# pyannote/pyannote-video

Hardware: AMD Instinct MI355X
Metric: frames/sec end-to-end detect->embed->cluster, 1080p@25fps (higher is better)
Workload: dtype f32 (detector scores, embedder) / f64 (tracker, clustering) / u8 frames; an f16 screening pass with a proven error bound decides which windows the detector's exact f32 chain is evaluated for -- results identical to dense f32 scoring (`dense_scoring`)

## Files before the change

pyannote-video_amd/csrc/api.hip:

```cpp
#include "pvf_internal.h"
#include <algorithm>
#include <cmath>
#include <cstdlib>
#include <string>
#include <thread>

#define API_BEGIN try {
#define API_END                                                        \
    return 0;                                                          \
    }                                                                  \
    catch (const std::exception& e) { pvf_set_error(e.what()); return -1; } \
    catch (...) { pvf_set_error("unknown error"); return -2; }

#define ENTER(c, h)                                                \
    Ctx* c = pvf_ctx(h);                                           \
    std::lock_guard<std::recursive_mutex> _api_lock(c->api_mu);    \
    HIP_CHECK(hipSetDevice(c->device))
#define ENTER_DET(c, h)                                            \
    Ctx* c = pvf_ctx(h);                                           \
    std::lock_guard<std::recursive_mutex> _det_lock(c->det_mu);    \
    HIP_CHECK(hipSetDevice(c->device))
#define ENTER_BOTH(c, h)                                           \
    Ctx* c = pvf_ctx(h);                                           \
    std::lock_guard<std::recursive_mutex> _det_lock(c->det_mu);    \
// ... 37 lines not shown
    API_BEGIN
    ENTER_DET(c, h);
    if (batches) *batches = c->screen_batches;
    if (listed) *listed = c->screen_listed;
    if (retries) *retries = c->screen_retries;
    if (bounds) for (int f = 0; f < c->det.n_filters; ++f) bounds[f] = c->det.screen_bound[f];
    if (pipe_err) *pipe_err = c->screen_pipe_err;
    API_END
}

extern "C" int32_t pvf_embedder_split(pvf_handle h, int32_t on)
{
    API_BEGIN
    ENTER(c, h);
    c->emb_split = on != 0;
    API_END
}

extern "C" int32_t pvf_embedder_split_stats(pvf_handle h, int64_t* faces, int64_t* reruns, double* pipe_err)
{
    API_BEGIN
    ENTER(c, h);
    if (faces) *faces = c->emb_split_faces;
    if (reruns) *reruns = c->emb_reruns;
    if (pipe_err) *pipe_err = c->emb_pipe_err;
    API_END
}

extern "C" int32_t pvf_detect_batch(pvf_handle h, const pvf_handle* frames, int32_t n_frames, int32_t upsample, double adjust,
                                    pvf_rect_i32* out, float* scores, int32_t* counts, int32_t cap)
// ... 762 lines not shown
        const size_t bytes = (size_t)n * 150 * 150 * 3;
        c->s_trk0.ensure(bytes);
        HIP_CHECK(hipMemcpyAsync(c->s_trk0.p, chips, bytes, hipMemcpyHostToDevice, c->stream));
    }
    resnet_debug_stage(c, c->s_trk0.as<uint8_t>(), n, split != 0, &tap, flags);
    for (int i = 0; i < 3; ++i) dims[i] = tap.dims[i];
    API_END
}

extern "C" int32_t pvf_debug_conv(pvf_handle h, const int32_t geom[18], const float* in, const float* w, const float* bias, const float* gamma,
                                  const float* beta, const float* skip, int32_t split, int32_t force_generic, float* out, int32_t* flags)
{
    API_BEGIN
    ENTER(c, h);
    PVF_REQUIRE(geom, "pvf_debug_conv: bad arguments");
    resnet_debug_conv(c, geom, in, w, bias, gamma, beta, skip, split != 0, force_generic != 0, out, flags);
    API_END
}

extern "C" int32_t pvf_debug_embed_head(pvf_handle h, const float* x, int32_t n, int32_t hw, float* out)
{
    API_BEGIN
    ENTER(c, h);
    resnet_debug_head(c, x, n, hw, out);
    API_END
}

static PairInput table_f64(const double* X) { PairInput in; in.X = X; return in; }
static PairOutput host_full(double* D) { PairOutput o; o.out = D; return o; }

extern "C" int32_t pvf_pair_mean_dist(pvf_handle h, const double* X, int32_t N, int32_t dim, const int32_t* row_start, int32_t T, double* D)
// ... 375 lines not shown
```

pyannote-video_amd/csrc/ctx.hip:

```cpp
#include "pvf_internal.h"
#include "detect_ml.h"
#include <cmath>
#include <fstream>
#include <mutex>
#include <dlfcn.h>

static thread_local std::string g_err;
void pvf_set_error(const char* msg) { g_err = msg ? msg : ""; }
extern "C" const char* pvf_last_error(void) { return g_err.c_str(); }

static std::mutex g_ctx_mu;
static std::unordered_map<uint64_t, std::unique_ptr<Ctx>> g_ctxs;
static uint64_t g_next_ctx = 0x1000;

Ctx* pvf_ctx(pvf_handle h)
{
    std::lock_guard<std::mutex> lk(g_ctx_mu);
    auto it = g_ctxs.find(h);
    if (it == g_ctxs.end()) throw PvfError("unknown context handle");
    return it->second.get();
}

std::map<std::string, Tensor> pvf_read_container(const char* path)
{
// ... 272 lines not shown
    if (strncmp(prop.gcnArchName, "gfx950", 6) != 0)
        throw PvfError(std::string("libpvface is built for gfx950 (MI355X) only; device is ") + prop.gcnArchName);
    std::unique_ptr<Ctx> c(new Ctx());
    c->device = device;
    c->n_cu = prop.multiProcessorCount;
    {
        int lo = 0, hi = 0;
        HIP_CHECK(hipDeviceGetStreamPriorityRange(&lo, &hi));
        int prio = priority_class < 0 ? lo : hi;
        if (const char* e = getenv("PVF_MAIN_STREAM_PRIO")) prio = (strcmp(e, "low") == 0) ? lo : hi;
        HIP_CHECK(hipStreamCreateWithPriority(&c->stream, hipStreamNonBlocking, priority_class == 2 ? lo : prio));
        HIP_CHECK(hipStreamCreateWithPriority(&c->det_stream, hipStreamNonBlocking, priority_class == 2 ? hi : lo));
    }
    if (const char* e = getenv("PVF_DETECTOR_SCREENING")) c->det_screen = atoi(e) != 0;
    if (const char* e = getenv("PVF_EMBEDDER_SPLIT")) c->emb_split = atoi(e) != 0;
    std::lock_guard<std::mutex> lk(g_ctx_mu);
    uint64_t id = g_next_ctx++;
    g_ctxs[id] = std::move(c);
    *out = id;
    API_END
}

extern "C" int32_t pvf_ctx_create(int32_t device, pvf_handle* out) { return pvf_ctx_create_prio(device, 0, out); }

extern "C" int32_t pvf_ctx_destroy(pvf_handle h)
{
    API_BEGIN
    Ctx* c = pvf_ctx(h);
    HIP_CHECK(hipSetDevice(c->device));
    (void)hipStreamSynchronize(c->stream);
// ... 259 lines not shown
```

pyannote-video_amd/csrc/pvf_internal.h:

```cpp
#pragma once
#include <hip/hip_runtime.h>
#include <cstdint>
#include <cstdio>
#include <cstring>
#include <deque>
#include <map>
#include <atomic>
#include <memory>
#include <mutex>
#include <stdexcept>
#include <string>
#include <unordered_map>
#include <vector>
#include "../../include/pvface.h"
#include "scratch_layout.h"
#include "chip_plan.h"
#include "group_blocks.h"

#define PVF_FHOG_STRIDE 32

struct CandOverflow : PvfError { int needed; explicit CandOverflow(int n) : PvfError("detector: candidate buffer overflow"), needed(n) {} };
struct ScreenRetry : PvfError { ScreenRetry() : PvfError("detector: screening pass gave up") {} };

#define HIP_CHECK(expr)                                                                              \
// ... 194 lines not shown
    HostBuf h_cand, h_misc;
    StageRing stage;
    DevBuf s_cand2[2], s_fptr[2];
    HostBuf h_cand2[2], h_fptr[2];
    hipEvent_t det_ev[2] = {nullptr, nullptr};
    int det_slot = 0;
    int det_cand_cap = 8192;
    bool det_screen = true, det_screen_suspended = false, screen_attr_set = false;
    int screen_list_cap = 1 << 20;
    DevBuf s_screen;
    int64_t screen_batches = 0, screen_listed = 0, screen_retries = 0;
    double screen_pipe_err = -1;
    bool screen_pipe_flushes_subnormals = false;
    bool emb_split = true, emb_probe_done = false;
    DevBuf s_emb_flags, s_emb_redo;
    DevBuf s_jit;
    bool jit_attr_set = false;
    int64_t emb_split_faces = 0, emb_reruns = 0;
    double emb_pipe_err = -1;
    int n_cu = 256;
    struct PoolBuf { uint8_t* p; hipEvent_t free_after; hipEvent_t free_after_det; };
    std::map<size_t, std::deque<PoolBuf>> frame_pool;
    size_t frame_pool_bytes = 0;
    void* ingest_rings = nullptr;
    void* render_state = nullptr;
    void* tube_state = nullptr;
    void* board_state = nullptr;
    struct MlPlanCache* ml_plans = nullptr;
    std::map<std::vector<int>, std::unique_ptr<DevBuf>> resize_tabs;
    const void* feat_ring_owner = nullptr;
// ... 110 lines not shown
void dlib_mean_face_shape(float* out );
void resnet_forward(Ctx* c, const uint8_t* d_chips, int n, float* h_out);
struct ChipSource { const uint8_t* host; const pvf_handle* frames; const int32_t* pts; };
const EmbedModel& faces_geometry();
void faces_make_chips(Ctx* c, const pvf_handle* frames, const int32_t* pts, int m, uint8_t* d_chips);
void faces_source_round(Ctx* c, const ChipSource& src, int i0, int m, uint8_t* d_chips);
void sheet_check(const std::string& w, int W, int H, uint32_t background, const pvf_prim* prims, int n_prims, const uint8_t* text,
                 int64_t text_bytes, const uint8_t* rgb);
void sheet_prims_launch(Ctx* c, const pvf_prim* d_prims, int n_prims, const uint8_t* d_text, int W, int H, uint8_t* d_rgb);
void conv_layer_upload(ConvLayer& L, const float* w, const float* bias, const float* gamma, const float* beta);
void conv_layer_free(ConvLayer& L);
#define EMB_STAGES 30
struct EmbedTap { int stage; float* h_out; int dims[3]; };
void resnet_debug_stage(Ctx* c, const uint8_t* d_chips, int n, bool split, EmbedTap* tap, int* h_flags);
void resnet_debug_conv(Ctx* c, const int32_t* geom, const float* in, const float* w, const float* bias, const float* gamma, const float* beta,
                       const float* skip, bool split, bool force_generic, float* out, int32_t* flags);
void resnet_debug_head(Ctx* c, const float* x, int n, int hw, float* out);
void dsst_start_many(Ctx* c, const std::vector<Tracker*>& t, const std::vector<Frame>& f, const double* boxes);
void dsst_clone_many(Ctx* c, const std::vector<Tracker*>& src, const std::vector<Tracker*>& dst);
double* tracker_state_alloc(Ctx* c);
void shot_dfd(Ctx* c, const std::vector<Frame>& frames, int ow, int oh, const float* tables22, double* dfd, uint8_t* gray_out, float* flow_out);
void shot_run(Ctx* c, const std::vector<Frame>& frames, int ow, int oh, const float* tables22, double* dfd, uint8_t* gray_out, float* flow_out,
              int64_t* motion_rows);
void motion_fit_device(Ctx* c, const float* d_flow, int n_pairs, int h, int w, const double* d_dfd, int64_t* d_rows);
std::vector<int> orb_level_quota();
void orb_extract(Ctx* c, const std::vector<Frame>& frames, int ow, int oh, int cap, int32_t* counts, float* kp_out, uint8_t* desc_out);
void orb_match_counts(Ctx* c, const uint8_t* desc, const int32_t* nrows, int n_sets, int cap, const int32_t* pairs, int64_t n_pairs, int32_t* out);
void dsst_update_many(Ctx* c, const std::vector<Tracker*>& t, const std::vector<Frame>& f, double* psr, double* boxes_out, int mode = 0);
void overlap_matrix_host(const double* a, int na, const double* b, int nb, double ratio, double* out);
void munkres_host(const double* cost, int n, int32_t* row_to_col);
struct PairInput {
// ... 32 lines not shown
```

pyannote-video_amd/csrc/resnet.hip:

```cpp
#include "pvf_internal.h"
#include <cmath>
#include <cstdlib>
#include <cstring>
#include <vector>

typedef float f32x4 __attribute__((ext_vector_type(4)));
typedef uint32_t u32x4 __attribute__((ext_vector_type(4)));
typedef float f32x16 __attribute__((ext_vector_type(16)));
typedef _Float16 f16x8 __attribute__((ext_vector_type(8)));
typedef _Float16 f16x4 __attribute__((ext_vector_type(4)));
typedef uint32_t u32x2 __attribute__((ext_vector_type(2)));

void face_chip_details(const EmbedModel& m, const int32_t* pts, ChipDetails* out)
{
    const double size = m.chip_size, padding = m.chip_padding;
    double fx[51], fy[51], tx[51], ty[51];
    int n = 0;
    for (int i = 17; i < 68; ++i) {
        if ((55 <= i && i <= 59) || (65 <= i && i <= 67)) continue;
        if (17 <= i && i <= 26) continue;
        fx[n] = ((padding + (double)m.mean_shape[2 * (i - 17)]) / (2 * padding + 1)) * size;
        fy[n] = ((padding + (double)m.mean_shape[2 * (i - 17) + 1]) / (2 * padding + 1)) * size;
        tx[n] = pts[2 * i]; ty[n] = pts[2 * i + 1];
        ++n;
// ... 18 lines not shown
    out->cs = ca / scale; out->sn = cb / scale;
    out->rows = m.chip_size; out->cols = m.chip_size;
}

struct ConvArgs {
    const float* in; int B, H, W, Cin;
    const float* w; int K;
    const float* frag;
    const float* bias; const float* gamma; const float* beta;
    float* out; int OH, OW, Cout;
    int AH, AW;
    int ksz, stride, pad;
    int skip_mode;
    const float* skip; int XH, XW, XC, SH, SW;
    const uint32_t* wsplit; float out_scale; int* flags;
};


__device__ __forceinline__ int small_div(int x, int d, float rd)
{
    int q = (int)((float)x * rd);
    const int r = x - q * d;
    q += (r >= d) ? 1 : 0;
    q -= (r < 0) ? 1 : 0;
    return q;
}

template <int WM, int WN>
__device__ __forceinline__ void conv_epilogue(const ConvArgs& a, float* smem, const f32x16& acc0, const f32x16& acc1, long M, long m0, int n0,
                                              int rel0, int b_first, int hw, float r_hw, float r_ow, int wave, int lane)
{
    constexpr int PITCH = 36;
// ... 13 lines not shown
        const float4 bias4 = *reinterpret_cast<const float4*>(a.bias + cb), g4 = *reinterpret_cast<const float4*>(a.gamma + cb),
                     bt4 = *reinterpret_cast<const float4*>(a.beta + cb);
#pragma unroll
        for (int it = 0; it < 8; ++it) {
            const int row = it * 8 + (lane >> 3);
            const long m = m0 + wm * 64 + row;
            if (m >= M) continue;
            const float4 x = *reinterpret_cast<const float4*>(&T[row * PITCH + 4 * c4]);
            float4 v = make_float4((x.x + bias4.x) * g4.x + bt4.x, (x.y + bias4.y) * g4.y + bt4.y, (x.z + bias4.z) * g4.z + bt4.z,
                                   (x.w + bias4.w) * g4.w + bt4.w);
            if (a.skip_mode == 1) {
                const float4 sk = *reinterpret_cast<const float4*>(a.skip + (size_t)m * a.Cout + cb);
                v.x += sk.x; v.y += sk.y; v.z += sk.z; v.w += sk.w;
            }
            { v.x = v.x < 0.0f ? 0.0f : v.x; v.y = v.y < 0.0f ? 0.0f : v.y; v.z = v.z < 0.0f ? 0.0f : v.z; v.w = v.w < 0.0f ? 0.0f : v.w; }
            *reinterpret_cast<float4*>(a.out + (size_t)m * a.Cout + cb) = v;
        }
        return;
    }
#pragma unroll
    for (int t = 0; t < 2; ++t)
#pragma unroll
        for (int reg = 0; reg < 16; ++reg) {
            const int row = (reg & 3) + 8 * (reg >> 2) + 4 * kh;
            const long m = m0 + wm * 64 + t * 32 + row;
            if (m >= M) continue;
            const int rel = rel0 + wm * 64 + t * 32 + row;
            const int bb = small_div(rel, hw, r_hw);
            const int rem = rel - bb * hw;
            const int oy = small_div(rem, a.OW, r_ow);
            const int ox = rem - oy * a.OW;
// ... 29 lines not shown
#pragma unroll
        for (int q = 0; q < 4; ++q) {
            fa0[q] = *reinterpret_cast<const f32x4*>(pa0 + 4 * q);
            fa1[q] = *reinterpret_cast<const f32x4*>(pa1 + 4 * q);
            fb[q] = *reinterpret_cast<const f32x4*>(pb + 4 * q);
        }
#pragma unroll
        for (int s = 0; s < 16; ++s) {
            acc0 = __builtin_amdgcn_mfma_f32_32x32x2f32(fa0[s >> 2][s & 3], fb[s >> 2][s & 3], acc0, 0, 0, 0);
            acc1 = __builtin_amdgcn_mfma_f32_32x32x2f32(fa1[s >> 2][s & 3], fb[s >> 2][s & 3], acc1, 0, 0, 0);
        }
    }
    static __device__ __forceinline__ void scale(const ConvArgs&, f32x16&, f32x16&) {}
};

#define EMB_A_SCALE_EXP 8
#define EMB_F16_LIMIT 65504.0f
struct ConvSplit {
    static constexpr bool FLAGS = true;
    static constexpr int LANE_K = 4;
    static __device__ __forceinline__ const u32x4* weights(const ConvArgs& a) { return reinterpret_cast<const u32x4*>(a.wsplit); }
    static __device__ __forceinline__ bool park_a(uint32_t* row, int j4, const u32x4& v)
    {
        const f32x4 xv = __builtin_bit_cast(f32x4, v) * (float)(1 << EMB_A_SCALE_EXP);
        const bool ok = __builtin_reduce_and(__builtin_elementwise_abs(xv) < EMB_F16_LIMIT);
        const f16x4 hi = __builtin_convertvector(xv, f16x4), lo = __builtin_convertvector(xv - __builtin_convertvector(hi, f32x4), f16x4);
        *reinterpret_cast<u32x2*>(row + 2 * j4) = __builtin_bit_cast(u32x2, hi);
        *reinterpret_cast<u32x2*>(row + 2 * j4 + 16) = __builtin_bit_cast(u32x2, lo);
        return ok;
    }
    static __device__ __forceinline__ void park_b(uint32_t* row, int j4, const u32x4& v) { *reinterpret_cast<u32x4*>(row + 4 * j4) = v; }
    static __device__ __forceinline__ void chunk(const uint32_t* pa0, const uint32_t* pa1, const uint32_t* pb, f32x16& acc0, f32x16& acc1)
    {
#pragma unroll
        for (int s = 0; s < 2; ++s) {
            const f16x8 ah0 = *reinterpret_cast<const f16x8*>(pa0 + 8 * s), al0 = *reinterpret_cast<const f16x8*>(pa0 + 16 + 8 * s);
            const f16x8 ah1 = *reinterpret_cast<const f16x8*>(pa1 + 8 * s), al1 = *reinterpret_cast<const f16x8*>(pa1 + 16 + 8 * s);
            const f16x8 bh = *reinterpret_cast<const f16x8*>(pb + 8 * s), bl = *reinterpret_cast<const f16x8*>(pb + 16 + 8 * s);
            acc0 = __builtin_amdgcn_mfma_f32_32x32x16_f16(ah0, bh, acc0, 0, 0, 0);
            acc1 = __builtin_amdgcn_mfma_f32_32x32x16_f16(ah1, bh, acc1, 0, 0, 0);
            acc0 = __builtin_amdgcn_mfma_f32_32x32x16_f16(ah0, bl, acc0, 0, 0, 0);
            acc1 = __builtin_amdgcn_mfma_f32_32x32x16_f16(ah1, bl, acc1, 0, 0, 0);
            acc0 = __builtin_amdgcn_mfma_f32_32x32x16_f16(al0, bh, acc0, 0, 0, 0);
            acc1 = __builtin_amdgcn_mfma_f32_32x32x16_f16(al1, bh, acc1, 0, 0, 0);
        }
    }
    static __device__ __forceinline__ void scale(const ConvArgs& a, f32x16& acc0, f32x16& acc1) { acc0 *= a.out_scale; acc1 *= a.out_scale; }
};

template <int WM, int WN, class Ops>
__global__ void __launch_bounds__(256) conv_tile_k(ConvArgs a)
{
    constexpr int BM = 64 * WM, BN = 32 * WN, KC = 32, PITCH = 36;
    static_assert(WM * WN == 4, "four waves per block");
    constexpr int SM_ROWS = (BM + BN > 256) ? BM + BN : 256;
    __shared__ __attribute__((aligned(16))) float smem[SM_ROWS * PITCH];
    uint32_t* As = reinterpret_cast<uint32_t*>(smem);
    uint32_t* Bs = As + BM * PITCH;
    const int tid = threadIdx.x, lane = tid & 63, wave = tid >> 6;
    const int wm = wave / WN, wn = wave % WN;
    const long M = (long)a.B * a.OH * a.OW;
    const long m0 = (long)blockIdx.x * BM;
// ... 94 lines not shown
}


__global__ void __launch_bounds__(256) conv_wsplit_k(const float* __restrict__ w, int total, int w_exp, _Float16* __restrict__ out)
{
    const int i = blockIdx.x * 256 + threadIdx.x;
    if (i >= total) return;
    const float v = ldexpf(w[i], w_exp);
    const _Float16 hi = (_Float16)v;
    const _Float16 lo = (_Float16)(v - (float)hi);
    const int row32 = i >> 5, kk = i & 31;
    out[(size_t)row32 * 64 + kk] = hi;
    out[(size_t)row32 * 64 + 32 + kk] = lo;
}

__global__ void __launch_bounds__(64) embed_probe_k(const uint4* __restrict__ a, const uint4* __restrict__ b, int steps, float* __restrict__ d)
{
    const int lane = threadIdx.x;
    f32x16 acc;
#pragma unroll
    for (int i = 0; i < 16; ++i) acc[i] = 0.0f;
    for (int s = 0; s < steps; ++s)
        acc = __builtin_amdgcn_mfma_f32_32x32x16_f16(__builtin_bit_cast(f16x8, a[s * 64 + lane]), __builtin_bit_cast(f16x8, b[s * 64 + lane]), acc, 0, 0, 0);
    for (int i = 0; i < 16; ++i) d[lane * 16 + i] = acc[i];
}

#define STEM_ROWS 4
#define STEM_IN_DW 1464
#define STEM_NP 77
__global__ void __launch_bounds__(64) stem_frag_k(const float* __restrict__ w, float* __restrict__ frag)
// ... 225 lines not shown
        out[(size_t)b * 128 + t] = acc;
    }
}

static bool conv_is_c32(const ConvArgs& a)
{
    return a.Cin == 32 && a.Cout == 32 && a.H == 35 && a.W == 35 && a.OH == 35 && a.OW == 35 && a.AH == 35 && a.AW == 35 && a.ksz == 3 &&
           a.stride == 1 && a.pad == 1 && a.skip_mode != 2;
}

static void launch_conv(Ctx* c, const ConvArgs& a)
{
    const long M = (long)a.B * a.OH * a.OW;
    PVF_REQUIRE(a.Cin % 32 == 0, "conv: input channels must be a multiple of 32 (the 3-channel first layer has a kernel of its own: stem_conv_k)");
    PVF_REQUIRE(a.OH * a.OW < (1 << 21) && a.Cout % 32 == 0, "conv: output map too large for the kernel's index arithmetic / Cout not a multiple of 32");
    auto tile = [&](auto exact, auto split, dim3 grid) { hipLaunchKernelGGL((a.wsplit ? split : exact), grid, dim3(256), 0, c->stream, a); };
    if (a.frag && conv_is_c32(a)) {
        static std::atomic<uint64_t> attr_set{0};
        const size_t lds = (size_t)(C32_TILE_FLOATS + 144 * 64) * sizeof(float);
        const uint64_t bit = 1ull << (c->device & 63);
        if (!(attr_set.load() & bit)) {
            HIP_CHECK(hipFuncSetAttribute(reinterpret_cast<const void*>(conv3x3_c32_k), hipFuncAttributeMaxDynamicSharedMemorySize, (int)lds));
            attr_set.fetch_or(bit);
        }
        const int items = a.B * (35 / C32_ROWS);
        hipLaunchKernelGGL(conv3x3_c32_k, dim3((unsigned)std::min(items, 2 * c->n_cu)), dim3(256), lds, c->stream, a.in, a.frag, a.bias, a.gamma, a.beta,
                           a.skip_mode == 1 ? a.skip : nullptr, a.out, items);
    } else if (a.Cout == 32) {
        tile(conv_tile_k<4, 1, ConvExact>, conv_tile_k<4, 1, ConvSplit>, dim3((unsigned)((M + 255) / 256), 1));
    } else {
        PVF_REQUIRE(a.Cout % 64 == 0, "conv: Cout must be 32 or a multiple of 64");
        tile(conv_tile_k<2, 2, ConvExact>, conv_tile_k<2, 2, ConvSplit>, dim3((unsigned)((M + 127) / 128), a.Cout / 64));
    }
}

void conv_layer_upload(ConvLayer& L, const float* w, const float* bias, const float* gamma, const float* beta)
{
    const int cin = L.cin, cout = L.cout, k = L.k;
    const int cp = (cin == 3) ? 4 : cin;
    const int K = k * k * cp, Kpad = (K + 31) / 32 * 32;
    std::vector<float> wt((size_t)cout * Kpad, 0.0f);
    for (int o = 0; o < cout; ++o)
        for (int ci = 0; ci < cin; ++ci)
            for (int r = 0; r < k; ++r)
                for (int s = 0; s < k; ++s) {
                    const int kk = (r * k + s) * cp + ci;
                    wt[(size_t)o * Kpad + kk] = w[(((size_t)o * cin + ci) * k + r) * k + s];
// ... 125 lines not shown
}

static void resnet_run(Ctx* c, const uint8_t* d_chips, int n, float* h_out, bool split, int* h_flags, const EmbedTap* tap = nullptr)
{
    const EmbedModel& e = c->emb;
    PVF_REQUIRE(e.loaded, "embedder not loaded");
    const int S = e.chip_size;
    const int MAXB = 4096;
    const int h1 = 1 + (S - 7) / 2;
    const int hp = 1 + (h1 - 3) / 2;
    const int cap = std::min(n, MAXB);
    const size_t big = (size_t)cap * h1 * h1 * 32;
    c->s_act0.ensure(std::max(big, (size_t)cap * S * S * 4) * sizeof(float));
    c->s_act1.ensure(big * sizeof(float));
    c->s_act2.ensure((size_t)cap * hp * hp * 32 * sizeof(float) + (size_t)cap * 128 * sizeof(float));
    PVF_REQUIRE(!tap || n <= MAXB, "embedder stage access: at most 4096 faces");
    auto tapped = [&](int stage, const float* d, int B, int H, int W, int C) {
        if (tap && tap->stage == stage && tap->h_out)
            HIP_CHECK(hipMemcpyAsync(tap->h_out, d, (size_t)B * H * W * C * sizeof(float), hipMemcpyDeviceToHost, c->stream));
    };
    for (int b0 = 0; b0 < n; b0 += MAXB) {
        const int B = std::min(MAXB, n - b0);
        ProfScope ps(c, "conv");
        float* x = c->s_act0.as<float>();
        float* y = c->s_act1.as<float>();
        float* z = c->s_act2.as<float>();
        const ConvLayer& L0 = e.convs[0];
        PVF_REQUIRE(S == 150 && L0.cout == 32 && L0.k == 7 && h1 == 72, "stem kernel: 150 x 150 chips, 7 x 7 stride 2, 32 channels");
        if (!c->emb.d_stem) {
            HIP_CHECK(hipMalloc(&c->emb.d_stem, STEM_NP * 64 * sizeof(float)));
// ... 1 lines not shown
        }
        hipLaunchKernelGGL(stem_conv_k, dim3(h1 / STEM_ROWS, B), dim3(192), 0, c->stream, d_chips + (size_t)b0 * S * S * 3, B, c->emb.d_stem,
                           L0.d_bias, L0.d_gamma, L0.d_beta, y);
        tapped(0, y, B, h1, h1, 32);
        ConvArgs a;
        const size_t npool = (size_t)B * hp * hp * 32;
        hipLaunchKernelGGL(maxpool3s2_k, dim3((unsigned)((npool + 255) / 256)), dim3(256), 0, c->stream, y, B, h1, h1, 32, z, hp, hp);
        tapped(1, z, B, hp, hp, 32);
        float* cur = z; float* t1 = x; float* t2 = y;
        int H = hp;
        int* flags = nullptr;
        if (split) {
            flags = c->s_emb_flags.as<int>();
            HIP_CHECK(hipMemsetAsync(flags, 0, (size_t)B * sizeof(int), c->stream));
        }
        for (int u = 0; u < 14; ++u) {
            const int cin = UN[u][0], nn = UN[u][1], down = UN[u][2];
            ConvLayer& La = c->emb.convs[1 + 2 * u];
            ConvLayer& Lb = c->emb.convs[2 + 2 * u];
            const int stride = down ? 2 : 1, pad = down ? 0 : 1;
            const auto [ah, sh, oh] = unit_dims(u, H);
            memset(&a, 0, sizeof a);
            a.in = cur; a.B = B; a.H = H; a.W = H; a.Cin = cin;
            a.out = t1; a.OH = ah; a.OW = ah; a.Cout = nn; a.AH = ah; a.AW = ah; a.ksz = 3; a.stride = stride; a.pad = pad; a.skip_mode = 0;
            conv_bind_weights(c, La, split, false, flags, a);
            launch_conv(c, a);
            tapped(2 + 2 * u, t1, B, ah, ah, nn);
            memset(&a, 0, sizeof a);
            a.in = t1; a.B = B; a.H = ah; a.W = ah; a.Cin = nn;
            a.out = t2; a.OH = oh; a.OW = oh; a.Cout = nn; a.AH = ah; a.AW = ah; a.ksz = 3; a.stride = 1; a.pad = 1;
            a.skip_mode = down ? 2 : 1; a.skip = cur; a.XH = H; a.XW = H; a.XC = cin; a.SH = sh; a.SW = sh;
            conv_bind_weights(c, Lb, split, false, flags, a);
            launch_conv(c, a);
            tapped(3 + 2 * u, t2, B, oh, oh, nn);
            float* old = cur; cur = t2; t2 = old;
            H = oh;
        }
        float* d_out = reinterpret_cast<float*>(c->s_act2.as<uint8_t>() + (size_t)cap * hp * hp * 32 * sizeof(float));
        hipLaunchKernelGGL(head_k, dim3(B), dim3(256), 0, c->stream, cur, H * H, e.d_fc, d_out);
        HIP_CHECK(hipGetLastError());
        HIP_CHECK(hipMemcpyAsync(h_out + (size_t)b0 * 128, d_out, (size_t)B * 128 * sizeof(float), hipMemcpyDeviceToHost, c->stream));
        if (split) HIP_CHECK(hipMemcpyAsync(h_flags + b0, flags, (size_t)B * sizeof(int), hipMemcpyDeviceToHost, c->stream));
    }
    HIP_CHECK(hipStreamSynchronize(c->stream));
}

void resnet_forward(Ctx* c, const uint8_t* d_chips, int n, float* h_out)
// ... 43 lines not shown
struct Scoped {
    void* p = nullptr;
    explicit Scoped(size_t bytes) { HIP_CHECK(hipMalloc(&p, bytes ? bytes : 4)); }
    ~Scoped() { if (p) (void)hipFree(p); }
    Scoped(const Scoped&) = delete;
    Scoped& operator=(const Scoped&) = delete;
};
struct ScopedLayer {
    ConvLayer L{};
    ~ScopedLayer() { conv_layer_free(L); }
};
struct Drain { Ctx* c; ~Drain() { (void)hipStreamSynchronize(c->stream); } };
}

void resnet_debug_conv(Ctx* c, const int32_t* g, const float* in, const float* w, const float* bias, const float* gamma, const float* beta,
                       const float* skip, bool split, bool force_generic, float* out, int32_t* flags)
{
    ConvArgs a;
    memset(&a, 0, sizeof a);
    a.B = g[0]; a.H = g[1]; a.W = g[2]; a.Cin = g[3]; a.OH = g[4]; a.OW = g[5]; a.Cout = g[6]; a.AH = g[7]; a.AW = g[8];
    a.ksz = g[9]; a.stride = g[10]; a.pad = g[11]; a.skip_mode = g[12]; a.XH = g[13]; a.XW = g[14]; a.XC = g[15]; a.SH = g[16]; a.SW = g[17];
    PVF_REQUIRE(in && w && bias && gamma && beta && out, "pvf_debug_conv: null tensor");
    PVF_REQUIRE(a.B > 0 && a.H > 0 && a.W > 0 && a.Cin > 0 && a.OH > 0 && a.OW > 0 && a.Cout > 0 && a.ksz > 0 && a.ksz <= 7 && a.stride > 0 && a.pad >= 0,
                "pvf_debug_conv: bad dimensions");
    PVF_REQUIRE(a.AH > 0 && a.AW > 0 && a.AH <= a.OH && a.AW <= a.OW, "pvf_debug_conv: the convolution's extent must lie inside the output map");
    PVF_REQUIRE(a.skip_mode >= 0 && a.skip_mode <= 2 && (a.skip_mode == 0 || skip), "pvf_debug_conv: skip_mode must be 0..2, with a skip tensor for 1 and 2");
    const size_t n_in = (size_t)a.B * a.H * a.W * a.Cin, n_out = (size_t)a.B * a.OH * a.OW * a.Cout;
    size_t n_skip = 0;
    if (a.skip_mode == 1) n_skip = n_out;
    if (a.skip_mode == 2) {
        PVF_REQUIRE(a.XH > 0 && a.XW > 0 && a.XC > 0 && a.SH >= 0 && a.SW >= 0 && 2 * a.SH <= a.XH && 2 * a.SW <= a.XW,
                    "pvf_debug_conv: the averaged skip map must lie inside the skip tensor");
        n_skip = (size_t)a.B * a.XH * a.XW * a.XC;
    }
    PVF_REQUIRE(n_in < (1u << 30) && n_out < (1u << 30) && n_skip < (1u << 30), "pvf_debug_conv: tensor too large");
    ScopedLayer sl;
    sl.L.cin = a.Cin; sl.L.cout = a.Cout; sl.L.k = a.ksz; sl.L.stride = a.stride; sl.L.pad = a.pad;
    conv_layer_upload(sl.L, w, bias, gamma, beta);
    Scoped d_in(n_in * sizeof(float)), d_out(n_out * sizeof(float)), d_skip(n_skip * sizeof(float));
    HIP_CHECK(hipMemcpyAsync(d_in.p, in, n_in * sizeof(float), hipMemcpyHostToDevice, c->stream));
    if (n_skip) HIP_CHECK(hipMemcpyAsync(d_skip.p, skip, n_skip * sizeof(float), hipMemcpyHostToDevice, c->stream));
    HIP_CHECK(hipMemsetAsync(d_out.p, 0xff, n_out * sizeof(float), c->stream));
    int* d_flags = nullptr;
    if (split) {
        c->s_emb_flags.ensure((size_t)a.B * sizeof(int));
        d_flags = c->s_emb_flags.as<int>();
        HIP_CHECK(hipMemsetAsync(d_flags, 0, (size_t)a.B * sizeof(int), c->stream));
    }
    a.in = reinterpret_cast<const float*>(d_in.p); a.out = reinterpret_cast<float*>(d_out.p);
    a.skip = n_skip ? reinterpret_cast<const float*>(d_skip.p) : nullptr;
    Drain drain{c};
    conv_bind_weights(c, sl.L, split, force_generic, d_flags, a);
    launch_conv(c, a);
    HIP_CHECK(hipGetLastError());
    HIP_CHECK(hipMemcpyAsync(out, d_out.p, n_out * sizeof(float), hipMemcpyDeviceToHost, c->stream));
    if (flags) {
        if (a.flags) HIP_CHECK(hipMemcpyAsync(flags, d_flags, (size_t)a.B * sizeof(int), hipMemcpyDeviceToHost, c->stream));
        else memset(flags, 0, (size_t)a.B * sizeof(int));
    }
    HIP_CHECK(hipStreamSynchronize(c->stream));
}

void resnet_debug_head(Ctx* c, const float* x, int n, int hw, float* out)
{
    PVF_REQUIRE(c->emb.loaded, "embedder not loaded");
    PVF_REQUIRE(x && out && n > 0 && hw > 0 && (size_t)n * hw < (1u << 22), "pvf_debug_embed_head: bad arguments");
    const size_t n_x = (size_t)n * hw * 256;
// ... 9 lines not shown
```

pyannote-video_amd/pyannote_video_amd/runtime.py:

```python
import contextlib
import ctypes as C
import threading
import itertools
import operator
import numpy as np
from . import _lib
from ._lib import check, ptr, handles
from . import models as _models
from .y4m import YuvFrame, chroma_shape


class DeviceFrame(object):
    __slots__ = ("ctx", "handle", "height", "width", "keep", "transient", "__weakref__")

    def __init__(self, ctx, handle, height, width, keep=None, transient=False):
        self.ctx, self.handle, self.height, self.width, self.keep = ctx, handle, height, width, keep
        self.transient = transient

    @property
    def shape(self):
        return (self.height, self.width, 3)

    def release(self):
        if self.handle is not None and self.ctx._h is not None:
# ... 781 lines not shown
        check(self._l.pvf_debug_extract_chip(self._h, f.handle, ptr(r), float(cs), float(sn), rows, cols, ptr(out)))
        return out

    EMBED_STAGES = 30

    def embed_stage(self, chips, stage, split):
        chips = np.ascontiguousarray(chips, np.uint8).reshape(-1, 150, 150, 3)
        n = len(chips)
        dims = np.zeros(3, np.int32)
        check(self._l.pvf_debug_embed_stage(self._h, None, n, 1 if split else 0, int(stage), None, ptr(dims), None))
        out = np.zeros((n,) + tuple(int(d) for d in dims), np.float32)
        flags = np.zeros(n, np.int32)
        check(self._l.pvf_debug_embed_stage(self._h, ptr(chips), n, 1 if split else 0, int(stage), ptr(out), ptr(dims), ptr(flags)))
        return out, flags

    def debug_conv(self, x, w, bias, gamma, beta, stride=1, pad=1, skip=None, skip_mode=0, out_hw=None, split=False, force_generic=False):
        x = np.ascontiguousarray(x, np.float32)
        w = np.ascontiguousarray(w, np.float32)
        B, H, W, cin = x.shape
        cout, wc, k, k2 = w.shape
        if wc != cin or k != k2:
            raise ValueError("debug_conv: weights do not fit the input")
        ah, aw = 1 + (H + 2 * pad - k) // stride, 1 + (W + 2 * pad - k) // stride
        xh = xw = xc = sh = sw = 0
        if skip is not None:
            skip = np.ascontiguousarray(skip, np.float32)
        if skip_mode == 2:
            _, xh, xw, xc = skip.shape
            sh, sw = xh // 2, xw // 2
        oh, ow = out_hw if out_hw is not None else (max(ah, sh), max(aw, sw))
        if skip_mode == 1 and skip.shape != (B, oh, ow, cout):
            raise ValueError("debug_conv: the skip tensor must have the output's shape")
        if skip_mode == 2 and skip.shape[0] != B:
            raise ValueError("debug_conv: one skip map per face")
        par = [np.ascontiguousarray(v, np.float32).reshape(-1) for v in (bias, gamma, beta)]
        if any(v.size != cout for v in par):
            raise ValueError("debug_conv: bias, gamma and beta have one value per output channel")
        geom = np.array([B, H, W, cin, oh, ow, cout, ah, aw, k, stride, pad, skip_mode, xh, xw, xc, sh, sw], np.int32)
        out = np.zeros((B, max(oh, 0), max(ow, 0), cout), np.float32)
        flags = np.zeros(B, np.int32)
        check(self._l.pvf_debug_conv(self._h, ptr(geom), ptr(x), ptr(w), ptr(par[0]), ptr(par[1]), ptr(par[2]),
                                     ptr(skip) if skip is not None else None, 1 if split else 0, 1 if force_generic else 0, ptr(out), ptr(flags)))
        return out, flags

    def embed_head(self, x):
        x = np.ascontiguousarray(x, np.float32)
        n, hw, ch = x.shape
        if ch != 256:
            raise ValueError("embed_head: 256 channels")
        out = np.zeros((n, 128), np.float32)
        check(self._l.pvf_debug_embed_head(self._h, ptr(x), n, hw, ptr(out)))
        return out

    def shot_dfd(self, frames, width, height, tables, want_gray=False, want_flow=False):
        n = len(frames)
        t = np.ascontiguousarray(tables, np.float32)
        if t.shape != (22,):
# ... 390 lines not shown
    def cluster_dist(self, D, row_start, threshold):
        return self._cluster_dist(D, row_start, threshold)[:2]

    def cluster_dist_cooccur(self, D, row_start, threshold, extent, flags=0):
        return self._cluster_dist(D, row_start, threshold, self._extent(extent, len(row_start) - 1), flags)

    def detector_screening(self, on=True, list_cap=0):
        check(self._l.pvf_detector_screening(self._h, 1 if on else 0, int(list_cap)))

    def detector_screening_stats(self):
        b, n, r, pe = C.c_int64(0), C.c_int64(0), C.c_int64(0), C.c_double(-1.0)
        bounds = np.zeros(8, np.float64)
        check(self._l.pvf_detector_screening_stats(self._h, C.byref(b), C.byref(n), C.byref(r), ptr(bounds), C.byref(pe)))
        return {"batches": b.value, "listed": n.value, "retries": r.value, "bounds": bounds[:5].tolist(), "pipe_err": pe.value}

    def embedder_split(self, on=True):
        check(self._l.pvf_embedder_split(self._h, 1 if on else 0))

    def embedder_split_stats(self):
        f, r, pe = C.c_int64(0), C.c_int64(0), C.c_double(-1.0)
        check(self._l.pvf_embedder_split_stats(self._h, C.byref(f), C.byref(r), C.byref(pe)))
        return {"faces": f.value, "reruns": r.value, "pipe_err": pe.value}

    def prof_enable(self, on=True):
        check(self._l.pvf_prof_enable(self._h, 1 if on else 0))

    def prof_reset(self):
        check(self._l.pvf_prof_reset(self._h))

    def prof_get(self, family):
        ms, n = C.c_double(0), C.c_int64(0)
        check(self._l.pvf_prof_get(self._h, family.encode(), C.byref(ms), C.byref(n)))
# ... 17 lines not shown
```

Baseline: 4785.

## Emit pre-split f16 hi/lo activations from conv epilogues for the next split conv

```diff
diff --git a/pyannote-video_amd/csrc/api.hip b/pyannote-video_amd/csrc/api.hip
--- a/pyannote-video_amd/csrc/api.hip
+++ b/pyannote-video_amd/csrc/api.hip
@@ -75,6 +75,7 @@
     API_BEGIN
     ENTER(c, h);
     c->emb_split = on != 0;
+    if (on == 2 || on == 3) c->emb_presplit = on == 3;
     API_END
 }
 
@@ -867,7 +868,7 @@
     API_BEGIN
     ENTER(c, h);
     PVF_REQUIRE(geom, "pvf_debug_conv: bad arguments");
-    resnet_debug_conv(c, geom, in, w, bias, gamma, beta, skip, split != 0, force_generic != 0, out, flags);
+    resnet_debug_conv(c, geom, in, w, bias, gamma, beta, skip, split != 0, force_generic, out, flags);
     API_END
 }
 
diff --git a/pyannote-video_amd/csrc/ctx.hip b/pyannote-video_amd/csrc/ctx.hip
--- a/pyannote-video_amd/csrc/ctx.hip
+++ b/pyannote-video_amd/csrc/ctx.hip
@@ -310,6 +310,7 @@
     }
     if (const char* e = getenv("PVF_DETECTOR_SCREENING")) c->det_screen = atoi(e) != 0;
     if (const char* e = getenv("PVF_EMBEDDER_SPLIT")) c->emb_split = atoi(e) != 0;
+    if (const char* e = getenv("PVF_EMBEDDER_PRESPLIT")) c->emb_presplit = atoi(e) != 0;
     std::lock_guard<std::mutex> lk(g_ctx_mu);
     uint64_t id = g_next_ctx++;
     g_ctxs[id] = std::move(c);
diff --git a/pyannote-video_amd/csrc/pvf_internal.h b/pyannote-video_amd/csrc/pvf_internal.h
--- a/pyannote-video_amd/csrc/pvf_internal.h
+++ b/pyannote-video_amd/csrc/pvf_internal.h
@@ -232,6 +232,8 @@
     bool screen_pipe_flushes_subnormals = false;
     bool emb_split = true, emb_probe_done = false;
     DevBuf s_emb_flags, s_emb_redo;
+    bool emb_presplit = true;
+    DevBuf s_spl_a, s_spl_u;
     DevBuf s_jit;
     bool jit_attr_set = false;
     int64_t emb_split_faces = 0, emb_reruns = 0;
@@ -372,7 +374,7 @@
 struct EmbedTap { int stage; float* h_out; int dims[3]; };
 void resnet_debug_stage(Ctx* c, const uint8_t* d_chips, int n, bool split, EmbedTap* tap, int* h_flags);
 void resnet_debug_conv(Ctx* c, const int32_t* geom, const float* in, const float* w, const float* bias, const float* gamma, const float* beta,
-                       const float* skip, bool split, bool force_generic, float* out, int32_t* flags);
+                       const float* skip, bool split, int mode, float* out, int32_t* flags);
 void resnet_debug_head(Ctx* c, const float* x, int n, int hw, float* out);
 void dsst_start_many(Ctx* c, const std::vector<Tracker*>& t, const std::vector<Frame>& f, const double* boxes);
 void dsst_clone_many(Ctx* c, const std::vector<Tracker*>& src, const std::vector<Tracker*>& dst);
diff --git a/pyannote-video_amd/csrc/resnet.hip b/pyannote-video_amd/csrc/resnet.hip
--- a/pyannote-video_amd/csrc/resnet.hip
+++ b/pyannote-video_amd/csrc/resnet.hip
@@ -56,8 +56,21 @@
     int skip_mode;
     const float* skip; int XH, XW, XC, SH, SW;
     const uint32_t* wsplit; float out_scale; int* flags;
+    bool in_split; uint32_t* out_split; int split_h, split_w;
 };
 
+
+#define EMB_A_SCALE_EXP 8
+#define EMB_F16_LIMIT 65504.0f
+__device__ __forceinline__ bool split_quad(const f32x4& x, u32x2& hi2, u32x2& lo2)
+{
+    const f32x4 xv = x * (float)(1 << EMB_A_SCALE_EXP);
+    const bool ok = __builtin_reduce_and(__builtin_elementwise_abs(xv) < EMB_F16_LIMIT);
+    const f16x4 hi = __builtin_convertvector(xv, f16x4), lo = __builtin_convertvector(xv - __builtin_convertvector(hi, f32x4), f16x4);
+    hi2 = __builtin_bit_cast(u32x2, hi);
+    lo2 = __builtin_bit_cast(u32x2, lo);
+    return ok;
+}
 
 __device__ __forceinline__ int small_div(int x, int d, float rd)
 {
@@ -101,7 +114,19 @@
                 v.x += sk.x; v.y += sk.y; v.z += sk.z; v.w += sk.w;
             }
             { v.x = v.x < 0.0f ? 0.0f : v.x; v.y = v.y < 0.0f ? 0.0f : v.y; v.z = v.z < 0.0f ? 0.0f : v.z; v.w = v.w < 0.0f ? 0.0f : v.w; }
-            *reinterpret_cast<float4*>(a.out + (size_t)m * a.Cout + cb) = v;
+            if (a.out) *reinterpret_cast<float4*>(a.out + (size_t)m * a.Cout + cb) = v;
+            if (a.out_split) {
+                u32x2 hi, lo;
+                const bool ok = split_quad(f32x4{v.x, v.y, v.z, v.w}, hi, lo);
+                *reinterpret_cast<u32x4*>(a.out_split + (size_t)m * a.Cout + cb) = u32x4{hi.x, hi.y, lo.x, lo.y};
+                if (!ok) {
+                    const int rel = rel0 + wm * 64 + row;
+                    const int bb = small_div(rel, hw, r_hw);
+                    const int rem = rel - bb * hw;
+                    const int oy = small_div(rem, a.OW, r_ow);
+                    if (oy < a.split_h && rem - oy * a.OW < a.split_w) a.flags[b_first + bb] = 1;
+                }
+            }
         }
         return;
     }
@@ -161,19 +186,16 @@
     static __device__ __forceinline__ void scale(const ConvArgs&, f32x16&, f32x16&) {}
 };
 
-#define EMB_A_SCALE_EXP 8
-#define EMB_F16_LIMIT 65504.0f
 struct ConvSplit {
     static constexpr bool FLAGS = true;
     static constexpr int LANE_K = 4;
     static __device__ __forceinline__ const u32x4* weights(const ConvArgs& a) { return reinterpret_cast<const u32x4*>(a.wsplit); }
     static __device__ __forceinline__ bool park_a(uint32_t* row, int j4, const u32x4& v)
     {
-        const f32x4 xv = __builtin_bit_cast(f32x4, v) * (float)(1 << EMB_A_SCALE_EXP);
-        const bool ok = __builtin_reduce_and(__builtin_elementwise_abs(xv) < EMB_F16_LIMIT);
-        const f16x4 hi = __builtin_convertvector(xv, f16x4), lo = __builtin_convertvector(xv - __builtin_convertvector(hi, f32x4), f16x4);
-        *reinterpret_cast<u32x2*>(row + 2 * j4) = __builtin_bit_cast(u32x2, hi);
-        *reinterpret_cast<u32x2*>(row + 2 * j4 + 16) = __builtin_bit_cast(u32x2, lo);
+        u32x2 hi, lo;
+        const bool ok = split_quad(__builtin_bit_cast(f32x4, v), hi, lo);
+        *reinterpret_cast<u32x2*>(row + 2 * j4) = hi;
+        *reinterpret_cast<u32x2*>(row + 2 * j4 + 16) = lo;
         return ok;
     }
     static __device__ __forceinline__ void park_b(uint32_t* row, int j4, const u32x4& v) { *reinterpret_cast<u32x4*>(row + 4 * j4) = v; }
@@ -193,6 +215,16 @@
         }
     }
     static __device__ __forceinline__ void scale(const ConvArgs& a, f32x16& acc0, f32x16& acc1) { acc0 *= a.out_scale; acc1 *= a.out_scale; }
+};
+
+struct ConvPre : ConvSplit {
+    static constexpr bool FLAGS = false;
+    static __device__ __forceinline__ bool park_a(uint32_t* row, int j4, const u32x4& v)
+    {
+        *reinterpret_cast<u32x2*>(row + 2 * j4) = u32x2{v.x, v.y};
+        *reinterpret_cast<u32x2*>(row + 2 * j4 + 16) = u32x2{v.z, v.w};
+        return true;
+    }
 };
 
 template <int WM, int WN, class Ops>
@@ -317,6 +349,15 @@
     out[(size_t)row32 * 64 + 32 + kk] = lo;
 }
 
+__global__ void __launch_bounds__(256) presplit_k(const f32x4* __restrict__ in, size_t quads, u32x4* __restrict__ out)
+{
+    const size_t i = (size_t)blockIdx.x * 256 + threadIdx.x;
+    if (i >= quads) return;
+    u32x2 hi, lo;
+    split_quad(in[i], hi, lo);
+    out[i] = u32x4{hi.x, hi.y, lo.x, lo.y};
+}
+
 __global__ void __launch_bounds__(64) embed_probe_k(const uint4* __restrict__ a, const uint4* __restrict__ b, int steps, float* __restrict__ d)
 {
     const int lane = threadIdx.x;
@@ -572,7 +613,13 @@
     const long M = (long)a.B * a.OH * a.OW;
     PVF_REQUIRE(a.Cin % 32 == 0, "conv: input channels must be a multiple of 32 (the 3-channel first layer has a kernel of its own: stem_conv_k)");
     PVF_REQUIRE(a.OH * a.OW < (1 << 21) && a.Cout % 32 == 0, "conv: output map too large for the kernel's index arithmetic / Cout not a multiple of 32");
-    auto tile = [&](auto exact, auto split, dim3 grid) { hipLaunchKernelGGL((a.wsplit ? split : exact), grid, dim3(256), 0, c->stream, a); };
+    PVF_REQUIRE(!(a.in_split || a.out_split) || (a.wsplit && a.flags), "conv: split tensors belong to the split form");
+    PVF_REQUIRE(a.out || a.out_split, "conv: no output tensor");
+    PVF_REQUIRE(!a.out_split || (a.AH == a.OH && a.AW == a.OW && a.skip_mode != 2 && !(a.frag && conv_is_c32(a))),
+                "conv: only the transposing store path writes a split tensor");
+    auto tile = [&](auto exact, auto split, auto pre, dim3 grid) {
+        hipLaunchKernelGGL((a.wsplit ? (a.in_split ? pre : split) : exact), grid, dim3(256), 0, c->stream, a);
+    };
     if (a.frag && conv_is_c32(a)) {
         static std::atomic<uint64_t> attr_set{0};
         const size_t lds = (size_t)(C32_TILE_FLOATS + 144 * 64) * sizeof(float);
@@ -585,10 +632,10 @@
         hipLaunchKernelGGL(conv3x3_c32_k, dim3((unsigned)std::min(items, 2 * c->n_cu)), dim3(256), lds, c->stream, a.in, a.frag, a.bias, a.gamma, a.beta,
                            a.skip_mode == 1 ? a.skip : nullptr, a.out, items);
     } else if (a.Cout == 32) {
-        tile(conv_tile_k<4, 1, ConvExact>, conv_tile_k<4, 1, ConvSplit>, dim3((unsigned)((M + 255) / 256), 1));
+        tile(conv_tile_k<4, 1, ConvExact>, conv_tile_k<4, 1, ConvSplit>, conv_tile_k<4, 1, ConvPre>, dim3((unsigned)((M + 255) / 256), 1));
     } else {
         PVF_REQUIRE(a.Cout % 64 == 0, "conv: Cout must be 32 or a multiple of 64");
-        tile(conv_tile_k<2, 2, ConvExact>, conv_tile_k<2, 2, ConvSplit>, dim3((unsigned)((M + 127) / 128), a.Cout / 64));
+        tile(conv_tile_k<2, 2, ConvExact>, conv_tile_k<2, 2, ConvSplit>, conv_tile_k<2, 2, ConvPre>, dim3((unsigned)((M + 127) / 128), a.Cout / 64));
     }
 }
 
@@ -744,6 +791,12 @@
     c->s_act0.ensure(std::max(big, (size_t)cap * S * S * 4) * sizeof(float));
     c->s_act1.ensure(big * sizeof(float));
     c->s_act2.ensure((size_t)cap * hp * hp * 32 * sizeof(float) + (size_t)cap * 128 * sizeof(float));
+    const bool presplit = split && c->emb_presplit;
+    const int h2 = 1 + (hp - 3) / 2;
+    if (presplit) {
+        c->s_spl_a.ensure((size_t)cap * h2 * h2 * 64 * sizeof(float));
+        c->s_spl_u.ensure((size_t)cap * h2 * h2 * 64 * sizeof(float));
+    }
     PVF_REQUIRE(!tap || n <= MAXB, "embedder stage access: at most 4096 faces");
     auto tapped = [&](int stage, const float* d, int B, int H, int W, int C) {
         if (tap && tap->stage == stage && tap->h_out)
@@ -775,6 +828,9 @@
             flags = c->s_emb_flags.as<int>();
             HIP_CHECK(hipMemsetAsync(flags, 0, (size_t)B * sizeof(int), c->stream));
         }
+        uint32_t* spl_a = presplit ? c->s_spl_a.as<uint32_t>() : nullptr;
+        uint32_t* spl_u = presplit ? c->s_spl_u.as<uint32_t>() : nullptr;
+        bool cur_split = false;
         for (int u = 0; u < 14; ++u) {
             const int cin = UN[u][0], nn = UN[u][1], down = UN[u][2];
             ConvLayer& La = c->emb.convs[1 + 2 * u];
@@ -785,6 +841,12 @@
             a.in = cur; a.B = B; a.H = H; a.W = H; a.Cin = cin;
             a.out = t1; a.OH = ah; a.OW = ah; a.Cout = nn; a.AH = ah; a.AW = ah; a.ksz = 3; a.stride = stride; a.pad = pad; a.skip_mode = 0;
             conv_bind_weights(c, La, split, false, flags, a);
+            const bool a_pre = presplit && a.wsplit;
+            if (cur_split) { a.in = reinterpret_cast<const float*>(spl_u); a.in_split = true; }
+            if (a_pre) {
+                a.out_split = spl_a; a.split_h = ah; a.split_w = ah;
+                if (!(tap && tap->stage == 2 + 2 * u && tap->h_out)) a.out = nullptr;
+            }
             launch_conv(c, a);
             tapped(2 + 2 * u, t1, B, ah, ah, nn);
             memset(&a, 0, sizeof a);
@@ -792,6 +854,12 @@
             a.out = t2; a.OH = oh; a.OW = oh; a.Cout = nn; a.AH = ah; a.AW = ah; a.ksz = 3; a.stride = 1; a.pad = 1;
             a.skip_mode = down ? 2 : 1; a.skip = cur; a.XH = H; a.XW = H; a.XC = cin; a.SH = sh; a.SW = sh;
             conv_bind_weights(c, Lb, split, false, flags, a);
+            if (a_pre) { a.in = reinterpret_cast<const float*>(spl_a); a.in_split = true; }
+            cur_split = a_pre && !down && u + 1 < 14;
+            if (cur_split) {
+                a.out_split = spl_u;
+                a.split_h = a.split_w = UN[u + 1][2] ? 2 * unit_dims(u + 1, oh).a + 1 : oh;
+            }
             launch_conv(c, a);
             tapped(3 + 2 * u, t2, B, oh, oh, nn);
             float* old = cur; cur = t2; t2 = old;
@@ -865,8 +933,11 @@
 }
 
 void resnet_debug_conv(Ctx* c, const int32_t* g, const float* in, const float* w, const float* bias, const float* gamma, const float* beta,
-                       const float* skip, bool split, bool force_generic, float* out, int32_t* flags)
-{
+                       const float* skip, bool split, int mode, float* out, int32_t* flags)
+{
+    const bool force_generic = mode & 1, pre_in = mode & 2, split_out = mode & 4;
+    const int extent = (mode >> 8) & 0xff;
+    PVF_REQUIRE(mode >= 0 && !(mode & ~0xff07) && (split || !(pre_in || split_out)) && (split_out || !extent), "pvf_debug_conv: bad mode");
     ConvArgs a;
     memset(&a, 0, sizeof a);
     a.B = g[0]; a.H = g[1]; a.W = g[2]; a.Cin = g[3]; a.OH = g[4]; a.OW = g[5]; a.Cout = g[6]; a.AH = g[7]; a.AW = g[8];
@@ -888,7 +959,7 @@
     ScopedLayer sl;
     sl.L.cin = a.Cin; sl.L.cout = a.Cout; sl.L.k = a.ksz; sl.L.stride = a.stride; sl.L.pad = a.pad;
     conv_layer_upload(sl.L, w, bias, gamma, beta);
-    Scoped d_in(n_in * sizeof(float)), d_out(n_out * sizeof(float)), d_skip(n_skip * sizeof(float));
+    Scoped d_in(n_in * sizeof(float)), d_out(n_out * sizeof(float)), d_skip(n_skip * sizeof(float)), d_in_split(pre_in ? n_in * sizeof(float) : 0);
     HIP_CHECK(hipMemcpyAsync(d_in.p, in, n_in * sizeof(float), hipMemcpyHostToDevice, c->stream));
     if (n_skip) HIP_CHECK(hipMemcpyAsync(d_skip.p, skip, n_skip * sizeof(float), hipMemcpyHostToDevice, c->stream));
     HIP_CHECK(hipMemsetAsync(d_out.p, 0xff, n_out * sizeof(float), c->stream));
@@ -902,6 +973,17 @@
     a.skip = n_skip ? reinterpret_cast<const float*>(d_skip.p) : nullptr;
     Drain drain{c};
     conv_bind_weights(c, sl.L, split, force_generic, d_flags, a);
+    PVF_REQUIRE(!(pre_in || split_out) || a.wsplit, "pvf_debug_conv: pre-split tensors belong to a layer of the split form");
+    if (pre_in) {
+        const size_t quads = n_in / 4;
+        hipLaunchKernelGGL(presplit_k, dim3((unsigned)((quads + 255) / 256)), dim3(256), 0, c->stream, reinterpret_cast<const f32x4*>(d_in.p), quads,
+                           reinterpret_cast<u32x4*>(d_in_split.p));
+        a.in = reinterpret_cast<const float*>(d_in_split.p); a.in_split = true;
+    }
+    if (split_out) {
+        a.out = nullptr; a.out_split = reinterpret_cast<uint32_t*>(d_out.p);
+        a.split_h = extent ? extent : a.OH; a.split_w = extent ? extent : a.OW;
+    }
     launch_conv(c, a);
     HIP_CHECK(hipGetLastError());
     HIP_CHECK(hipMemcpyAsync(out, d_out.p, n_out * sizeof(float), hipMemcpyDeviceToHost, c->stream));
diff --git a/pyannote-video_amd/pyannote_video_amd/runtime.py b/pyannote-video_amd/pyannote_video_amd/runtime.py
--- a/pyannote-video_amd/pyannote_video_amd/runtime.py
+++ b/pyannote-video_amd/pyannote_video_amd/runtime.py
@@ -819,7 +819,8 @@
         check(self._l.pvf_debug_embed_stage(self._h, ptr(chips), n, 1 if split else 0, int(stage), ptr(out), ptr(dims), ptr(flags)))
         return out, flags
 
-    def debug_conv(self, x, w, bias, gamma, beta, stride=1, pad=1, skip=None, skip_mode=0, out_hw=None, split=False, force_generic=False):
+    def debug_conv(self, x, w, bias, gamma, beta, stride=1, pad=1, skip=None, skip_mode=0, out_hw=None, split=False, force_generic=False,
+                   presplit=False, split_out=False, read_extent=0):
         x = np.ascontiguousarray(x, np.float32)
         w = np.ascontiguousarray(w, np.float32)
         B, H, W, cin = x.shape
@@ -841,11 +842,14 @@
         par = [np.ascontiguousarray(v, np.float32).reshape(-1) for v in (bias, gamma, beta)]
         if any(v.size != cout for v in par):
             raise ValueError("debug_conv: bias, gamma and beta have one value per output channel")
+        mode = (1 if force_generic else 0) | (2 if presplit else 0) | (4 if split_out else 0) | (int(read_extent) << 8)
         geom = np.array([B, H, W, cin, oh, ow, cout, ah, aw, k, stride, pad, skip_mode, xh, xw, xc, sh, sw], np.int32)
         out = np.zeros((B, max(oh, 0), max(ow, 0), cout), np.float32)
         flags = np.zeros(B, np.int32)
         check(self._l.pvf_debug_conv(self._h, ptr(geom), ptr(x), ptr(w), ptr(par[0]), ptr(par[1]), ptr(par[2]),
-                                     ptr(skip) if skip is not None else None, 1 if split else 0, 1 if force_generic else 0, ptr(out), ptr(flags)))
+                                     ptr(skip) if skip is not None else None, 1 if split else 0, mode, ptr(out), ptr(flags)))
+        if split_out:
+            out = out.view(np.float16).reshape(B, max(oh, 0), max(ow, 0), cout // 4, 2, 4)
         return out, flags
 
     def embed_head(self, x):
@@ -1266,8 +1270,8 @@
         check(self._l.pvf_detector_screening_stats(self._h, C.byref(b), C.byref(n), C.byref(r), ptr(bounds), C.byref(pe)))
         return {"batches": b.value, "listed": n.value, "retries": r.value, "bounds": bounds[:5].tolist(), "pipe_err": pe.value}
 
-    def embedder_split(self, on=True):
-        check(self._l.pvf_embedder_split(self._h, 1 if on else 0))
+    def embedder_split(self, on=True, presplit=None):
+        check(self._l.pvf_embedder_split(self._h, (1 if presplit is None else 3 if presplit else 2) if on else 0))
 
     def embedder_split_stats(self):
         f, r, pe = C.c_int64(0), C.c_int64(0), C.c_double(-1.0)
```

After: 4801 (median of 4 runs). No clear change (+0.3%).
